# pmvreeswijk/BlackBOX

Hardware: AMD Instinct MI355X
Metric: 10560x10560 fp32 frames/sec end-to-end reduce+ZOGY; % HBM roofline (higher is better)
Workload: dtype f32

## Files before the change

### blackbox_amd/csrc/bbx_canny.hip

```cpp
#include "bbx_common.h"

#define CANNY_MAXR 32

struct canny_par {
    unsigned prefix[4];
    unsigned long long rank[4];
    double p1, p2, low, high;
    float p1f, p2f, den;
    int degenerate;
    double w[CANNY_MAXR + 1];
    int radius;
};

__global__ void k_canny_init(canny_par* p, size_t n, double q1, double q2, const double* __restrict__ w, int radius, unsigned* hist) {
    const int t = threadIdx.x;
    for (int i = t; i < 4 * 4096; i += blockDim.x) hist[i] = 0;
    if (t <= radius) p->w[t] = w[t];
    if (t == 0) {
        const double v1 = (double)(n - 1) * q1, v2 = (double)(n - 1) * q2;
        const unsigned long long l1 = (unsigned long long)floor(v1), l2 = (unsigned long long)floor(v2);
        p->rank[0] = l1; p->rank[1] = l1 + 1 < n ? l1 + 1 : n - 1;
        p->rank[2] = l2; p->rank[3] = l2 + 1 < n ? l2 + 1 : n - 1;
        for (int q = 0; q < 4; q++) p->prefix[q] = 0;
        p->radius = radius; p->degenerate = 0;
    }
}

template <int PASS>
__global__ __launch_bounds__(256) void k_canny_hist(const float* __restrict__ b, size_t n, const canny_par* __restrict__ p,
                                                    unsigned* __restrict__ hist) {
    __shared__ unsigned h[4096];
    for (int i = threadIdx.x; i < 4096; i += blockDim.x) h[i] = 0;
    __syncthreads();
    unsigned pre[4];
#pragma unroll
    for (int q = 0; q < 4; q++) pre[q] = p->prefix[q];
    const size_t n4 = n >> 2, stride = (size_t)gridDim.x * blockDim.x;
    const float4* b4 = (const float4*)b;
    auto count = [&](float f) {
        const unsigned k = f2key(f);
        if (PASS == 0) {
            const unsigned bin = k >> 20;
            bool pending = true;
#pragma unroll
            for (int r = 0; r < 2; r++) {
                const unsigned long long act = __builtin_amdgcn_ballot_w64(pending);
                if (!act) break;
                const int leader = (int)__builtin_ctzll(act);
                const unsigned b0 = (unsigned)__builtin_amdgcn_readlane((int)bin, leader);
                const bool same = pending && bin == b0;
                const unsigned long long m = __builtin_amdgcn_ballot_w64(same);
                if ((int)(threadIdx.x & 63) == leader) atomicAdd(&h[b0], (unsigned)__popcll(m));
                pending = pending && !same;
            }
            if (pending) atomicAdd(&h[bin], 1u);
        } else {
#pragma unroll
            for (int q = 0; q < 4; q++) {
                if (q > 0 && pre[q] == pre[q - 1]) continue;
                if (PASS == 1 && (k >> 20) == pre[q]) atomicAdd(&h[q * 1024 + ((k >> 10) & 1023u)], 1u);
                if (PASS == 2 && (k >> 10) == pre[q]) atomicAdd(&h[q * 1024 + (k & 1023u)], 1u);
            }
        }
    };
    for (size_t i = (size_t)blockIdx.x * blockDim.x + threadIdx.x; i < n4; i += stride) {
        const float4 f = b4[i];
        count(f.x); count(f.y); count(f.z); count(f.w);
    }
    if (blockIdx.x == 0 && threadIdx.x < (n & 3)) count(b[n4 * 4 + threadIdx.x]);
    __syncthreads();
    for (int i = threadIdx.x; i < 4096; i += blockDim.x) if (h[i]) atomicAdd(&hist[i], h[i]);
}

template <int PASS>
__global__ __launch_bounds__(256) void k_canny_scan(canny_par* p, unsigned* hist) {
    __shared__ unsigned sh[4096];
    for (int i = threadIdx.x; i < 4096; i += blockDim.x) sh[i] = hist[i];
    __syncthreads();
    const int q = threadIdx.x >> 6, lane = threadIdx.x & 63;
    int qh = q;
    if (PASS != 0) { while (qh > 0 && p->prefix[qh] == p->prefix[qh - 1]) qh--; }
    __syncthreads();
    const unsigned* h = PASS == 0 ? sh : sh + qh * 1024;
    constexpr int NB = PASS == 0 ? 4096 : 1024, CH = NB / 64;
    unsigned long long mine = 0;
    for (int i = 0; i < CH; i++) mine += h[lane * CH + i];
    unsigned long long incl = mine;
#pragma unroll
// ... 164 lines not shown
        }
        __syncthreads();
        const unsigned nc = ncand;
        for (unsigned t = tid; t < nc; t += 256) {
            const int i = s_cand[t];
            const int ty = i / CT_X, tx = i - ty * CT_X, y = y0 + ty, x = x0 + tx;
            const int r = ty + 1, c = tx + 1;
            double is, js;
            grad(r, c, is, js);
            const double m = sqrt(is * is + js * js);
            if (!(m > 0.0 && m >= low)) continue;
            const double ai = fabs(is), aj = fabs(js);
            const bool same = (is >= 0 && js >= 0) || (is <= 0 && js <= 0), opp = (is <= 0 && js >= 0) || (is >= 0 && js <= 0);
            int sec = 0;
            if (same && ai >= aj) sec = 1;
            if (same && ai <= aj) sec = 2;
            if (opp && ai <= aj) sec = 3;
            if (opp && ai >= aj) sec = 4;
            if (!sec) continue;
            const int dr2 = sec <= 2 ? 1 : -1, dr1 = (sec == 1) ? 1 : (sec == 4 ? -1 : 0), dc1 = (sec == 2 || sec == 3) ? 1 : 0;
            const double w = (sec == 1 || sec == 4) ? aj / ai : ai / aj;
            const bool loc = (mag(r + dr2, c + 1) * w + mag(r + dr1, c + dc1) * (1 - w) <= m) &&
                             (mag(r - dr2, c - 1) * w + mag(r - dr1, c - dc1) * (1 - w) <= m);
            if (loc) { const unsigned k = atomicAdd(&qn, 1u); q[k] = (uint32_t)((size_t)y * nx + x) | (m >= high ? 0x80000000u : 0u); }
        }
        __syncthreads();
        if (tid == 0) ncand = 0;
    }
}

int bbx_cc_filter_list(bbx_ctx* ctx, const uint32_t* d_list, const int32_t* d_cnt, size_t cap, int ny, int nx, const uint8_t* d_flag,
                       int min_size, uint32_t* d_out, int32_t* d_out_cnt, uint32_t out_cap, hipStream_t s);

int bbx_canny_edges(bbx_ctx* ctx, const float* d_bin, int ny, int nx, const double* h_gauss, int radius, double low_frac, double high_frac,
                    int min_size, uint32_t* d_out, int32_t* d_out_cnt, uint32_t out_cap, hipStream_t s) {
    if (radius < 1 || radius > CANNY_MAXR || ny < 3 || nx < 3) return BBX_ERR_ARG;
    const size_t n = (size_t)ny * nx;
    int rc;
    const size_t cap = n / 8 + 4096;
    const size_t o_par = 0, o_hist = 4096, o_w = o_hist + 4 * 4096 * 4, o_tmp = o_w + 1024;
    const size_t o_sm = o_tmp + ((n * 4 + 255) & ~(size_t)255);
    const size_t o_list = o_sm + ((n * 8 + 255) & ~(size_t)255), o_flag = o_list + ((cap * 4 + 255) & ~(size_t)255);
    const size_t total = o_flag + cap + 256;
    char* ws = (char*)bbx_ws(ctx, WS_CANNY, total, &rc); if (rc) return rc;
    canny_par* par = (canny_par*)(ws + o_par); unsigned* hist = (unsigned*)(ws + o_hist); double* d_w = (double*)(ws + o_w);
    float* tmp = (float*)(ws + o_tmp); double* sm = (double*)(ws + o_sm);
    uint32_t* list = (uint32_t*)(ws + o_list); uint8_t* hflag = (uint8_t*)(ws + o_flag);
    int32_t* cnt = &ctx->d_counters[CNT_TMP];
    const double q1 = 4.5 / 100.0, q2 = 93.0 / 100.0;
    BBX_HIP(hipMemcpyAsync(d_w, h_gauss, (size_t)(radius + 1) * 8, hipMemcpyHostToDevice, s));
    BBX_HIP(hipMemsetAsync(cnt, 0, sizeof(int32_t), s));
#ifdef SATV
    const int satv = getenv("BBX_DBG_SAT") ? atoi(getenv("BBX_DBG_SAT")) : 0;
    if (satv >= 5) return BBX_OK;
#endif
    hipLaunchKernelGGL(k_canny_init, dim3(1), dim3(256), 0, s, par, n, q1, q2, d_w, radius, hist);
    hipLaunchKernelGGL(k_canny_hist<0>, dim3(1024), dim3(256), 0, s, d_bin, n, par, hist);
    hipLaunchKernelGGL(k_canny_scan<0>, dim3(1), dim3(256), 0, s, par, hist);
    hipLaunchKernelGGL(k_canny_hist<1>, dim3(1024), dim3(256), 0, s, d_bin, n, par, hist);
    hipLaunchKernelGGL(k_canny_scan<1>, dim3(1), dim3(256), 0, s, par, hist);
    hipLaunchKernelGGL(k_canny_hist<2>, dim3(1024), dim3(256), 0, s, d_bin, n, par, hist);
    hipLaunchKernelGGL(k_canny_scan<2>, dim3(1), dim3(256), 0, s, par, hist);
    hipLaunchKernelGGL(k_canny_params, dim3(1), dim3(64), 0, s, par, n, q1, q2, low_frac, high_frac);
    const dim3 gx((nx + 255) / 256, (ny + GH_ROWS - 1) / GH_ROWS), gv((nx + 255) / 256, (ny + GV_RY - 1) / GV_RY);
#ifdef SATV
    if (satv >= 4) return BBX_OK;
#endif
    if (radius == 12) {
        hipLaunchKernelGGL(k_canny_gauss_v<12>, gv, dim3(256), 0, s, d_bin, ny, nx, par, tmp);
        hipLaunchKernelGGL(k_canny_gauss_h<12>, gx, dim3(256), 0, s, tmp, ny, nx, par, sm);
    } else {
        return BBX_ERR_ARG;
    }
#ifdef SATV
    if (satv >= 3) return BBX_OK;
#endif
    hipLaunchKernelGGL(k_canny_tile, dim3((nx + CT_X - 1) / CT_X, (ny + CT_Y * CT_NT - 1) / (CT_Y * CT_NT)), dim3(256), 0, s, sm, ny, nx, par, list, hflag, cnt,
                       (uint32_t)cap, ctx->d_err);
    BBX_LAUNCH_CHECK();
#ifdef SATV
    if (satv >= 2) return BBX_OK;
#endif
    return bbx_cc_filter_list(ctx, list, cnt, cap, ny, nx, hflag, min_size, d_out, d_out_cnt, out_cap, s);
}

__global__ __launch_bounds__(256) void k_canny_scatter(const uint32_t* __restrict__ list, const int32_t* __restrict__ cnt, uint32_t cap,
                                                       uint8_t* __restrict__ map) {
    const uint32_t n = min((uint32_t)*cnt, cap);
    for (uint32_t e = blockIdx.x * blockDim.x + threadIdx.x; e < n; e += gridDim.x * blockDim.x) map[list[e]] = 1;
}

extern "C" int bbx_canny_edge_map(bbx_ctx* ctx, int ny, int nx, const float* d_img, const double* h_gauss, int gauss_radius,
                                  double low_frac, double high_frac, int min_size, uint8_t* d_map, int32_t* d_count, void* stream) {
    if (!ctx || !d_img || !h_gauss || !d_map || !d_count || ((uintptr_t)d_img) % 16) return BBX_ERR_ARG;
    hipStream_t s = (hipStream_t)stream;
    int rc;
    const size_t n = (size_t)ny * nx, cap = n / 8 + 4096;
    uint32_t* out = (uint32_t*)bbx_ws(ctx, WS_CRLIST, cap * sizeof(uint32_t), &rc); if (rc) return rc;
    BBX_HIP(hipMemsetAsync(d_map, 0, n, s));
    rc = bbx_canny_edges(ctx, d_img, ny, nx, h_gauss, gauss_radius, low_frac, high_frac, min_size, out, d_count, (uint32_t)cap, s);
    if (rc) return rc;
    hipLaunchKernelGGL(k_canny_scatter, dim3(256), dim3(256), 0, s, out, d_count, (uint32_t)cap, d_map);
    BBX_LAUNCH_CHECK();
    return BBX_OK;
}

int bbx_build_flags_canny(void) {
#ifdef SATV
    return 8;
#else
    return 0;
#endif
}
```

### blackbox_amd/csrc/bbx_common.h

```cpp
#pragma once
#include <hip/hip_runtime.h>
#include <hip/hip_ext.h>
#include <stdint.h>
#include <stdio.h>
#include <string.h>
#include "../../include/bbx.h"

#define BBX_WAVE 64

struct bbx_dims {
    int ny_raw, nx_raw, ysz, xsz;
    int dy, dx;
    int os_y, os_x;
    int vos_x0, vos_w;
    int hos_rows;
    int ny, nx;
};

static inline int bbx_make_dims(const bbx_geom* g, bbx_dims* d) {
    if (!g || g->ny_raw <= 0 || g->nx_raw <= 0 || g->ysize_chan <= 0 || g->xsize_chan <= 0)
        return BBX_ERR_ARG;
    d->ny_raw = g->ny_raw; d->nx_raw = g->nx_raw;
    d->ysz = g->ysize_chan; d->xsz = g->xsize_chan;
    if (d->ny_raw % 2 || d->nx_raw % 8) return BBX_ERR_ARG;
    d->dy = d->ny_raw / 2; d->dx = d->nx_raw / 8;
    d->os_y = (d->ny_raw - 2 * d->ysz) / 2;
    d->os_x = (d->nx_raw - 8 * d->xsz) / 8;
    if (d->os_y != d->dy - d->ysz || d->os_x != d->dx - d->xsz) return BBX_ERR_ARG;
    d->hos_rows = d->os_y - 10;
    d->vos_x0 = d->xsz + 5;
    d->vos_w = d->dx - 1 - d->vos_x0;
    if (d->hos_rows <= 0 || d->vos_w <= 0) return BBX_ERR_ARG;
    d->ny = 2 * d->ysz; d->nx = 8 * d->xsz;
    return BBX_OK;
}

#define BBX_DERR_LIST_OVERFLOW 1
#define BBX_DERR_NOTCONV       2
#define BBX_DERR_PSF_WINDOW    4

struct bbx_zprep { const float2* buf; const void* id[2]; int S; int geom[4]; };

struct bbx_ctx {
    int device;
    char hip_err[256];
    int32_t* d_err;
    uint32_t* d_satlist;  int64_t cap_satlist;
    void*     flags_clean_ptr;
    size_t    flags_clean_bytes;
    void*     d_nonlin;
    int       nonlin_on;
    void*     hash_clean_ptr;
    size_t    hash_clean_n;
    int32_t*  d_counters;
    void*  d_ws[24];
    size_t ws_bytes[24];
    int    lac_feed;
    int    debug_listcap;
    void*  zogy_state;
    void*  zogy_frame_state;
    int    zogy_kwin_off;
    int    zogy_ksmall_off;
    int    sat_attr_set;
    int    mini_attr_set;
    float  zcand_thr;
    const float* zcand_img;
    float  zcand_thr_used; size_t zcand_npix;
    bbx_zprep zrows;
    bbx_zprep zpsf;
    const float* bcand_med;
    double bcand_nsig;
    const float* bcand_img;
    const float* bcand_img_med; double bcand_img_nsig; size_t bcand_npix;
    int    wait_sleep_us;
    int    cc_roots;
    int    box_pp;
    int    bkg_full_sort;
    int    fpack_hist_only;
    struct { void* stream; void* ptr; size_t bytes; } fphint[16];
    int    fpack_one_wg;
    int    spf_attr_bytes;
    int    zogy3_attr_L;
    int    num_cus;
    int prof_on, prof_n;
    volatile int prof_gen;
    int prof_open, prof_open_gen, prof_open_idx;
    hipEvent_t* prof_ev;
    int* prof_slot;
};
#define BBX_PROF_MAX 8192
void bbx_prof_start(bbx_ctx* ctx, int slot, hipStream_t s);
void bbx_prof_stop(bbx_ctx* ctx, hipStream_t s);
void bbx_prof_events(bbx_ctx* ctx, int slot, hipEvent_t* e0, hipEvent_t* e1);
#define BBX_LAUNCH_TIMED(ctx, slot, kern, grid, blk, lds, s, ...)                                   \
    do {                                                                                              \
        hipEvent_t e0_ = nullptr, e1_ = nullptr;                                                      \
        bbx_prof_events(ctx, slot, &e0_, &e1_);                                                       \
        hipExtLaunchKernelGGL(kern, grid, blk, lds, s, e0_, e1_, 0, __VA_ARGS__);                     \
    } while (0)

enum {
    CNT_SAT = 0,
    CNT_CAND = 16,
    CNT_STAGE2 = 32,
    CNT_CRLIST = 48,
    CNT_NEWCR = 64,
    CNT_CC_N = 80,
    CNT_CC_ROOTS = 96,
    CNT_TILES = 112,
    CNT_BGNEED = 128,
    CNT_TMP = 144,
    CNT_CANDOVF = 160,
    CNT_CANDRAW = 176,
    CNT_TICKET = 192,
    CNT_ZCAND = 208,
    CNT_BCAND = 224,
    CNT_BOXFAIL0 = 240,
    CNT_MAX = 256
};

enum {
    WS_HASH = 0, WS_CCLIST, WS_PARENT, WS_BITS_M, WS_BITS_C, WS_BITS_R, WS_TILES,
    WS_CAND, WS_FLAGS, WS_STAGE2, WS_CRLIST, WS_HIST, WS_SEL, WS_MISC, WS_STRIP, WS_HVALS, WS_CRORIG, WS_CANNY, WS_ZCAND, WS_BCAND, WS_FPHINT, WS_BOXFAIL, WS_ZSPL,
    WS_TRANSFIT,
    WS_MAX
};

int bbx_hip_fail(bbx_ctx* ctx, hipError_t e, const char* what, int line);
static inline size_t bbx_cand_cap(size_t npix) {
    const size_t c = npix / 16 + 1024, f = npix < 65536 ? npix : 65536;
    return c > f ? c : f;
}
void bbx_zogy_frame_release(bbx_ctx* ctx);
void bbx_fpack_release(bbx_ctx* ctx);
int bbx_build_flags_fpack(void); int bbx_build_flags_zogy(void); int bbx_build_flags_bkg(void); int bbx_build_flags_sat(void); int bbx_build_flags_canny(void);
void bbx_zogy_release(bbx_ctx* ctx);
void* bbx_ws(bbx_ctx* ctx, int slot, size_t bytes, int* rc);

struct f32x16 { float v[16]; };
struct f64x256 { double v[256]; };

#define BBX_HIP(call)                                                         \
    do {                                                                      \
        hipError_t _e = (call);                                               \
        if (_e != hipSuccess) return bbx_hip_fail(ctx, _e, #call, __LINE__);  \
    } while (0)

#define BBX_LAUNCH_CHECK()                                                    \
    do {                                                                      \
        hipError_t _e = hipGetLastError();                                    \
        if (_e != hipSuccess) return bbx_hip_fail(ctx, _e, "kernel launch", __LINE__); \
    } while (0)

template <int CTRL> __device__ __forceinline__ int dpp_mov_i32(int v) {
    return __builtin_amdgcn_update_dpp(0, v, CTRL, 0xf, 0xf, false);
}
template <int CTRL> __device__ __forceinline__ float dpp_mov_f32(float v) {
    return __int_as_float(dpp_mov_i32<CTRL>(__float_as_int(v)));
}
template <int CTRL> __device__ __forceinline__ double dpp_mov_f64(double v) {
    const int lo = dpp_mov_i32<CTRL>(__double2loint(v)), hi = dpp_mov_i32<CTRL>(__double2hiint(v));
    return __hiloint2double(hi, lo);
}
__device__ __forceinline__ double readlane_f64(double v, int lane) {
    return __hiloint2double(__builtin_amdgcn_readlane(__double2hiint(v), lane), __builtin_amdgcn_readlane(__double2loint(v), lane));
}
__device__ __forceinline__ float readlane_f32(float v, int lane) { return __int_as_float(__builtin_amdgcn_readlane(__float_as_int(v), lane)); }
#define BBX_DPP_ROR(n) (0x120 + (n))
__device__ __forceinline__ double wave_sum_f64(double v) {
    v += dpp_mov_f64<BBX_DPP_ROR(1)>(v);
// ... 31 lines not shown
        if (lane == leader) atomicAdd(&size[r0], (unsigned)__popcll(same));
        on = on && root != r0;
        m &= ~same;
    }
}

__device__ __forceinline__ bool finite_f32(float v) { return (__float_as_uint(v) & 0x7f800000u) != 0x7f800000u; }

__device__ __forceinline__ unsigned atomic_or_u8(uint8_t* base, size_t idx, unsigned bits) {
    size_t a = (size_t)(base + idx);
    unsigned* w = (unsigned*)(a & ~(size_t)3);
    unsigned sh = (unsigned)(a & 3) * 8;
    unsigned old = atomicOr(w, bits << sh);
    return (old >> sh) & 0xffu;
}
__device__ __forceinline__ void atomic_clear_u8(uint8_t* base, size_t idx, unsigned bits) {
    size_t a = (size_t)(base + idx);
    atomicAnd((unsigned*)(a & ~(size_t)3), ~(bits << ((unsigned)(a & 3) * 8)));
}

template <int RAW_T>
__device__ __forceinline__ float raw_load(const void* raw, size_t i) {
    if (RAW_T == BBX_RAW_U16) return (float)((const uint16_t*)raw)[i];
    return ((const float*)raw)[i];
}

__device__ __forceinline__ uint32_t f2key(float f) {
    uint32_t u = __float_as_uint(f);
    return (u & 0x80000000u) ? ~u : (u | 0x80000000u);
}
__device__ __forceinline__ float key2f(uint32_t k) {
    uint32_t u = (k & 0x80000000u) ? (k & 0x7fffffffu) : ~k;
    return __uint_as_float(u);
}

__device__ __forceinline__ uint32_t umed3(uint32_t a, uint32_t b, uint32_t c) {
    uint32_t o;
    asm("v_med3_u32 %0, %1, %2, %3" : "=v"(o) : "v"(a), "v"(b), "v"(c));
    return o;
}
template <int NR, int K, int J> __device__ __forceinline__ void wave_sort_static(uint32_t (&k)[NR]) {
#pragma unroll
    for (int r = 0; r < NR; r++) {
        const int q = r ^ J;
        if (q > r) {
            const uint32_t a = k[r], b = k[q];
            const uint32_t lo = min(a, b), hi = max(a, b);
            if ((r & K) == 0) { k[r] = lo; k[q] = hi; } else { k[r] = hi; k[q] = lo; }
        }
    }
}
template <int NR, int J> __device__ __forceinline__ void wave_sort_lane(uint32_t (&k)[NR], uint32_t clo) {
    const uint32_t chi = ~clo;
#pragma unroll
    for (int r = 0; r < NR; r++) {
        const int q = r ^ J;
        if (q > r) {
            const uint32_t a = k[r], b = k[q];
            k[r] = umed3(a, b, clo); k[q] = umed3(a, b, chi);
        }
    }
}
template <int NR> __device__ __forceinline__ void wave_sort_cross(uint32_t (&k)[NR], int lane, int m, bool asc) {
    const uint32_t c = (((lane & m) == 0) == asc) ? 0u : 0xffffffffu;
#pragma unroll
    for (int r = 0; r < NR; r++) k[r] = umed3(k[r], (uint32_t)__shfl_xor((int)k[r], m), c);
// ... 102 lines not shown
```

### blackbox_amd/csrc/bbx_ctx.hip

```cpp
#include "bbx_common.h"
#include <stdlib.h>
#include <time.h>

int bbx_hip_fail(bbx_ctx* ctx, hipError_t e, const char* what, int line) {
    if (ctx)
        snprintf(ctx->hip_err, sizeof(ctx->hip_err), "%s: %s (line %d)", what,
                 hipGetErrorString(e), line);
    (void)hipGetLastError();
    return BBX_ERR_HIP;
}

void* bbx_ws(bbx_ctx* ctx, int slot, size_t bytes, int* rc) {
    *rc = BBX_OK;
    if (slot < 0 || slot >= WS_MAX) { *rc = BBX_ERR_ARG; return nullptr; }
    if (ctx->ws_bytes[slot] >= bytes && ctx->d_ws[slot]) return ctx->d_ws[slot];
    if (ctx->d_ws[slot]) {
        (void)hipDeviceSynchronize();
        (void)hipFree(ctx->d_ws[slot]);
        ctx->d_ws[slot] = nullptr; ctx->ws_bytes[slot] = 0;
    }
    size_t want = bytes + bytes / 8 + 256;
    hipError_t e = hipMalloc(&ctx->d_ws[slot], want);
    if (e != hipSuccess) { *rc = bbx_hip_fail(ctx, e, "hipMalloc(workspace)", __LINE__); return nullptr; }
    ctx->ws_bytes[slot] = want;
    return ctx->d_ws[slot];
}

void bbx_prof_start(bbx_ctx* ctx, int slot, hipStream_t s) {
    ctx->prof_open = 0;
    if (!ctx->prof_on || ctx->prof_n >= BBX_PROF_MAX) return;
    const int n = ctx->prof_n;
    ctx->prof_open_gen = ctx->prof_gen;
    ctx->prof_slot[n] = slot;
    (void)hipEventRecord(ctx->prof_ev[2 * n], s);
    ctx->prof_open = 1; ctx->prof_open_idx = n;
}
void bbx_prof_events(bbx_ctx* ctx, int slot, hipEvent_t* e0, hipEvent_t* e1) {
    *e0 = *e1 = nullptr;
    ctx->prof_open = 0;
    if (!ctx->prof_on || ctx->prof_n >= BBX_PROF_MAX) return;
    const int n = ctx->prof_n;
    ctx->prof_slot[n] = slot;
    *e0 = ctx->prof_ev[2 * n]; *e1 = ctx->prof_ev[2 * n + 1];
    ctx->prof_n = n + 1;
}
void bbx_prof_stop(bbx_ctx* ctx, hipStream_t s) {
    if (!ctx->prof_open) return;
    ctx->prof_open = 0;
    if (!ctx->prof_on || ctx->prof_open_gen != ctx->prof_gen || ctx->prof_open_idx != ctx->prof_n) return;
    (void)hipEventRecord(ctx->prof_ev[2 * ctx->prof_n + 1], s);
    ctx->prof_n++;
}

#define BBX_HIP0(call) do { if ((call) != hipSuccess) return BBX_ERR_HIP; } while (0)

extern "C" {

int bbx_version(void) { return 100; }
// ... 47 lines not shown

int bbx_ctx_create(int device, bbx_ctx** out) {
    if (!out) return BBX_ERR_ARG;
    *out = nullptr;
    bbx_ctx* ctx = (bbx_ctx*)calloc(1, sizeof(bbx_ctx));
    if (!ctx) return BBX_ERR_NOMEM;
    ctx->device = device;
    hipError_t e = hipSetDevice(device);
    if (e == hipSuccess) e = hipMalloc((void**)&ctx->d_err, 4 * sizeof(int32_t));
    if (e == hipSuccess) e = hipMemset(ctx->d_err, 0, 4 * sizeof(int32_t));
    if (e == hipSuccess) e = hipMalloc((void**)&ctx->d_counters, CNT_MAX * sizeof(int32_t));
    if (e == hipSuccess) e = hipMemset(ctx->d_counters, 0, CNT_MAX * sizeof(int32_t));
    ctx->num_cus = 0;
    if (e == hipSuccess) e = hipDeviceGetAttribute(&ctx->num_cus, hipDeviceAttributeMultiprocessorCount, device);
    if (e != hipSuccess) {
        fprintf(stderr, "bbx_ctx_create: %s\n", hipGetErrorString(e));
        free(ctx);
        return BBX_ERR_HIP;
    }
    *out = ctx;
    return BBX_OK;
}

void bbx_ctx_destroy(bbx_ctx* ctx) {
    if (!ctx) return;
    (void)hipSetDevice(ctx->device);
    (void)hipDeviceSynchronize();
    bbx_zogy_release(ctx);
    bbx_zogy_frame_release(ctx);
    bbx_fpack_release(ctx);
    for (int i = 0; i < WS_MAX; i++) if (ctx->d_ws[i]) (void)hipFree(ctx->d_ws[i]);
    if (ctx->d_satlist) (void)hipFree(ctx->d_satlist);
    if (ctx->d_nonlin) (void)hipFree(ctx->d_nonlin);
    if (ctx->d_err) (void)hipFree(ctx->d_err);
    if (ctx->d_counters) (void)hipFree(ctx->d_counters);
    if (ctx->prof_ev) { for (int i = 0; i < 2 * BBX_PROF_MAX; i++) (void)hipEventDestroy(ctx->prof_ev[i]); free(ctx->prof_ev); free(ctx->prof_slot); }
    free(ctx);
}

__global__ __launch_bounds__(256) void k_copy_bytes(const uint8_t* __restrict__ src, uint8_t* __restrict__ dst, size_t n, int words) {
    const size_t i0 = (size_t)blockIdx.x * blockDim.x + threadIdx.x, step = (size_t)gridDim.x * blockDim.x;
    if (words) {
        const size_t nw = n >> 2;
        for (size_t i = i0; i < nw; i += step) reinterpret_cast<uint32_t*>(dst)[i] = reinterpret_cast<const uint32_t*>(src)[i];
        for (size_t i = (nw << 2) + i0; i < n; i += step) dst[i] = src[i];
    } else {
        for (size_t i = i0; i < n; i += step) dst[i] = src[i];
    }
}

int bbx_copy_kernel(void* dst, const void* src, size_t nbytes, void* stream) {
    if (!dst || !src) return BBX_ERR_ARG;
    if (nbytes == 0) return BBX_OK;
    const int words = (((uintptr_t)dst | (uintptr_t)src) & 3) == 0;
    const size_t items = words ? (nbytes >> 2) + 3 : nbytes;
    const int blocks = (int)((items + 255) / 256 < 1024 ? (items + 255) / 256 : 1024);
    hipLaunchKernelGGL(k_copy_bytes, dim3(blocks), dim3(256), 0, (hipStream_t)stream, (const uint8_t*)src, (uint8_t*)dst, nbytes, words);
    if (hipGetLastError() != hipSuccess) return BBX_ERR_HIP;
    return BBX_OK;
}

static int bbx_poll_event(hipEvent_t ev, int sleep_us) {
    struct timespec ts; ts.tv_sec = 0; ts.tv_nsec = (long)sleep_us * 1000L;
    for (;;) {
        const hipError_t e = hipEventQuery(ev);
        if (e == hipSuccess) return BBX_OK;
// ... 29 lines not shown
    int32_t* err = g_wait.h_err;
    err[0] = 0;
    BBX_HIP(hipMemcpyAsync(err, ctx->d_err, 4 * sizeof(int32_t), hipMemcpyDeviceToHost, (hipStream_t)stream));
    { const int rc = bbx_wait(ctx, stream); if (rc) return rc; }
    if (err[0]) {
        BBX_HIP(hipMemsetAsync(ctx->d_err, 0, 4 * sizeof(int32_t), (hipStream_t)stream));
        if (err[0] & BBX_DERR_PSF_WINDOW) return BBX_ERR_PSFWIN;
        if (err[0] & BBX_DERR_LIST_OVERFLOW) return BBX_ERR_OVERFLOW;
        if (err[0] & BBX_DERR_NOTCONV) return BBX_ERR_NOTCONV;
    }
    return BBX_OK;
}

__global__ void k_step_mark(int32_t* err, int32_t* slot) { *slot = err[0]; err[0] = 0; }

int bbx_step_mark(bbx_ctx* ctx, int32_t* d_slot, void* stream) {
    if (!ctx || !d_slot) return BBX_ERR_ARG;
    hipLaunchKernelGGL(k_step_mark, dim3(1), dim3(1), 0, (hipStream_t)stream, ctx->d_err, d_slot);
    BBX_LAUNCH_CHECK();
    return BBX_OK;
}

int bbx_set_option(bbx_ctx* ctx, int option, int value) {
    if (!ctx) return BBX_ERR_ARG;
    if (option == BBX_OPT_LAC_LEVEL_FEED) { ctx->lac_feed = value ? 1 : 0; return BBX_OK; }
    if (option == BBX_OPT_ZOGY_CORE) return BBX_OK;
    if (option == BBX_OPT_DEBUG_LISTCAP) { ctx->debug_listcap = value > 0 ? value : 0; return BBX_OK; }
    if (option == BBX_OPT_ZOGY_KWIN_OFF) { ctx->zogy_kwin_off = value ? 1 : 0; return BBX_OK; }
    if (option == BBX_OPT_ZOGY_KSMALL_OFF) { ctx->zogy_ksmall_off = value ? 1 : 0; return BBX_OK; }
    if (option == BBX_OPT_FPACK_ONE_WG) { ctx->fpack_one_wg = value ? 1 : 0; return BBX_OK; }
    if (option == BBX_OPT_FPACK_HIST_ONLY) { ctx->fpack_hist_only = value ? 1 : 0; return BBX_OK; }
    if (option == BBX_OPT_BKG_FULL_SORT) { ctx->bkg_full_sort = value ? 1 : 0; return BBX_OK; }
    if (option == BBX_OPT_WAIT_SLEEP_US) { ctx->wait_sleep_us = value > 0 ? value : 0; return BBX_OK; }
    return BBX_ERR_ARG;
}


int bbx_event_create(void** out_event) {
    if (!out_event) return BBX_ERR_ARG;
    hipEvent_t ev;
    BBX_HIP0(hipEventCreateWithFlags(&ev, hipEventDisableTiming));
    *out_event = (void*)ev;
    return BBX_OK;
}

void bbx_event_destroy(void* event) {
    if (event) (void)hipEventDestroy((hipEvent_t)event);
}

int bbx_event_record(void* event, void* stream) {
    if (!event) return BBX_ERR_ARG;
    BBX_HIP0(hipEventRecord((hipEvent_t)event, (hipStream_t)stream));
    return BBX_OK;
}

int bbx_event_query(void* event) {
    if (!event) return BBX_ERR_ARG;
    const hipError_t e = hipEventQuery((hipEvent_t)event);
    if (e == hipSuccess) return 1;
    if (e == hipErrorNotReady) { (void)hipGetLastError(); return 0; }
    return BBX_ERR_HIP;
}

int bbx_stream_wait_event(void* stream, void* event) {
    if (!event) return BBX_ERR_ARG;
    BBX_HIP0(hipStreamWaitEvent((hipStream_t)stream, (hipEvent_t)event, 0));
// ... 13 lines not shown
```

### blackbox_amd/csrc/bbx_sat.hip

```cpp
#include "bbx_common.h"

#define SAT_BLOCKS 1024

struct sat_state {
    unsigned long long best;
    int accept, found, k, lo_off, hi_off;
    int votes;
    double rho, c, s, chord;
    unsigned long long tmin, tmax;
    double t0, t1;
    unsigned long long fit_n; long long fit_t, fit_d, fit_tt, fit_td;
    double icpt, slope;
    unsigned int bmax_key, bmin_key;
    int seg[4], seg_ok;
    double m[6], m2[6];
    int rot_rows, rot_cols, back_rows, back_cols, crop_y, crop_x;
    double sx, sy;
    double top, clip_lo, clip_hi;
    int band_r0, band_rows;
    int nwin, row_min, row_max;
};
#define SAT_BANDH 96
#define SAT_MAXWIN 1200
#define SAT_SEG_CAP 8192
#define SAT_SUBLEN 5
#define SAT_SUBW 200
struct sat_rect { int r0, r1, c0, c1; };


__global__ __launch_bounds__(256) void k_bin2(const float* __restrict__ d, int nyb, int nxb, float* __restrict__ b) {
    const int X = blockIdx.x * blockDim.x + threadIdx.x, Y = blockIdx.y;
    if (X >= nxb) return;
    const size_t nx = (size_t)nxb * 2;
    const float2 r0 = *(const float2*)(d + (size_t)(2 * Y) * nx + 2 * X);
    const float2 r1 = *(const float2*)(d + (size_t)(2 * Y + 1) * nx + 2 * X);
    b[(size_t)Y * nxb + X] = (r0.x + r0.y) + (r1.x + r1.y);
}

__global__ __launch_bounds__(256) void k_bin_minmax(const float* __restrict__ b, size_t n, sat_state* st) {
    unsigned hi = 0u, lo = ~0u;
    const size_t n4 = n >> 2, stride = (size_t)gridDim.x * blockDim.x;
    const float4* b4 = (const float4*)b;
    for (size_t i = (size_t)blockIdx.x * blockDim.x + threadIdx.x; i < n4; i += stride) {
        const float4 q = b4[i];
        const float f[4] = {q.x, q.y, q.z, q.w};
#pragma unroll
        for (int u = 0; u < 4; u++) if (isfinite(f[u])) { const unsigned k = f2key(f[u]); hi = k > hi ? k : hi; lo = k < lo ? k : lo; }
    }
    if (blockIdx.x == 0 && threadIdx.x < (n & 3)) { const float f = b[(n4 << 2) + threadIdx.x]; if (isfinite(f)) { const unsigned k = f2key(f); hi = k > hi ? k : hi; lo = k < lo ? k : lo; } }
    for (int o = 32; o > 0; o >>= 1) { const unsigned a = __shfl_xor(hi, o, 64), c = __shfl_xor(lo, o, 64); hi = a > hi ? a : hi; lo = c < lo ? c : lo; }
    __shared__ unsigned shi[4], slo[4];
    if ((threadIdx.x & 63) == 0) { shi[threadIdx.x >> 6] = hi; slo[threadIdx.x >> 6] = lo; }
    __syncthreads();
    if (threadIdx.x == 0) {
        for (int w = 1; w < 4; w++) { hi = shi[w] > hi ? shi[w] : hi; lo = slo[w] < lo ? slo[w] : lo; }
        if (hi) { atomicMax(&st->bmax_key, hi); atomicMin(&st->bmin_key, lo); }
    }
}

__global__ void k_sat_init(sat_state* st) {
    if (threadIdx.x == 0) {
        st->best = 0;
        st->accept = 0; st->found = 0; st->k = 0; st->lo_off = 0; st->hi_off = 0; st->votes = 0;
        st->rho = 0; st->c = 0; st->s = 0; st->chord = 0; st->tmin = ~0ull; st->tmax = 0ull; st->t0 = 0; st->t1 = 0;
        st->fit_n = 0; st->fit_t = st->fit_d = st->fit_tt = st->fit_td = 0; st->icpt = 0; st->slope = 0;
        st->bmax_key = 0u; st->bmin_key = ~0u; st->seg_ok = 0; st->nwin = 0; st->row_min = 0x7fffffff; st->row_max = -1;
        st->band_r0 = 0; st->band_rows = 0; st->rot_rows = st->rot_cols = 0;
    }
}

__global__ __launch_bounds__(1024) void k_hough_lds(const uint32_t* __restrict__ list, const int32_t* __restrict__ cnt, uint32_t cap,
                                                    int nxb, const double* __restrict__ cs, int nrho, sat_state* st) {
    extern __shared__ unsigned hist[];
    const int k = blockIdx.x;
    const uint32_t n = min((uint32_t)*cnt, cap);
    for (int i = threadIdx.x; i < nrho; i += blockDim.x) hist[i] = 0;
    __syncthreads();
    const double c = cs[2 * k], s = cs[2 * k + 1];
    const int off = nrho / 2;
    for (uint32_t e = threadIdx.x; e < n; e += blockDim.x) {
        const uint32_t p = list[e];
        const double y = (double)(p / nxb), x = (double)(p % nxb);
        const double r = c * x + s * y;
        atomicAdd(&hist[(int)(r > 0.0 ? r + 0.5 : r - 0.5) + off], 1u);
    }
    __syncthreads();
    unsigned long long best = 0;
    for (int i = threadIdx.x; i < nrho; i += blockDim.x) {
        const unsigned v = hist[i];
        const unsigned long long flat = (unsigned long long)k * nrho + i;
// ... 392 lines not shown
        const double fminr = floor(r), fminc = floor(c);
        const long long minr = (long long)fminr, minc = (long long)fminc, maxr = (long long)ceil(r), maxc = (long long)ceil(c);
        const double dr = r - fminr, dc = c - fminc;
        double p[4];
        const long long rr[4] = {minr, minr, maxr, maxr}, cc[4] = {minc, maxc, minc, maxc};
        for (int q = 0; q < 4; q++) {
            double v = 0.0;
            if (rr[q] >= 0 && rr[q] < rot_rows && cc[q] >= 0 && cc[q] < rot_cols)
                for (int w = 0; w < nwin; w++)
                    if (rr[q] >= R[w].r0 && rr[q] < R[w].r1 && cc[q] >= R[w].c0 && cc[q] < R[w].c1) { v = 1.0; break; }
            p[q] = v;
        }
        const double top = (1 - dc) * p[0] + dc * p[1], bot = (1 - dc) * p[2] + dc * p[3];
        const double out = (1 - dr) * top + dr * bot;
        if (out != 0.0) {
            uint16_t* a = reinterpret_cast<uint16_t*>(mask + (size_t)(2 * Y) * nx + 2 * X);
            uint16_t* bq = reinterpret_cast<uint16_t*>(mask + (size_t)(2 * Y + 1) * nx + 2 * X);
            *a |= (uint16_t)(BBX_MASK_SATELLITE | (BBX_MASK_SATELLITE << 8));
            *bq |= (uint16_t)(BBX_MASK_SATELLITE | (BBX_MASK_SATELLITE << 8));
        }
    }
}

__global__ void k_sat_info(const sat_state* __restrict__ st, float* info) {
    if (threadIdx.x == 0) {
        info[0] = key2f(st->bmax_key); info[1] = key2f(st->bmin_key); info[2] = (float)st->votes; info[3] = (float)st->k;
        info[4] = (float)st->rho; info[5] = (float)st->nwin; info[6] = (float)st->seg_ok; info[7] = (float)st->found;
    }
}

extern "C" int bbx_count_objects(bbx_ctx* ctx, int ny, int nx, const uint8_t* d_mask, int bit, int32_t* d_count, void* stream);

int bbx_canny_edges(bbx_ctx* ctx, const float* d_bin, int ny, int nx, const double* h_gauss, int radius, double low_frac, double high_frac,
                    int min_size, uint32_t* d_out, int32_t* d_out_cnt, uint32_t out_cap, hipStream_t s);

extern "C" int bbx_sat_trails(bbx_ctx* ctx, int ny, int nx, const float* d_data, uint8_t* d_mask, const double* h_cos_sin,
                              int ntheta, const double* h_gauss, int gauss_radius, int32_t* d_nsats, float* d_info, void* stream) {
    if (!ctx || !d_data || !d_mask || !h_cos_sin || !h_gauss || !d_nsats || !d_info || ny < 8 || nx < 8 || (ny & 1) || (nx & 1) ||
        ntheta < 4 || ntheta > 4096 || ((uintptr_t)d_data) % 8)
        return BBX_ERR_ARG;
    hipStream_t s = (hipStream_t)stream;
    const int nyb = ny / 2, nxb = nx / 2;
    const size_t nb = (size_t)nyb * nxb;
    const int nrho = 2 * (int)ceil(sqrt((double)nyb * nyb + (double)nxb * nxb));
    int rc;
    const size_t cap = nb / 8 + 4096;
    const size_t o_bin = 0, o_list = o_bin + ((nb * 4 + 255) & ~(size_t)255);
    const size_t o_cs = o_list + ((cap * 4 + 255) & ~(size_t)255), o_part = o_cs + (((size_t)ntheta * 16 + 255) & ~(size_t)255);
    const size_t o_st = o_part + SAT_BLOCKS * 3 * 8;
    const int band_cols = nrho / 2 + 8;
    const size_t o_rect = (o_st + sizeof(sat_state) + 255) & ~(size_t)255, o_band = (o_rect + SAT_MAXWIN * sizeof(sat_rect) + 255) & ~(size_t)255;
    const size_t total = o_band + (size_t)2 * SAT_BANDH * band_cols * sizeof(double) + 256;
    char* ws = (char*)bbx_ws(ctx, WS_CAND, total, &rc); if (rc) return rc;
    float* bin = (float*)(ws + o_bin); uint32_t* list = (uint32_t*)(ws + o_list);
    double* cs = (double*)(ws + o_cs); sat_state* st = (sat_state*)(ws + o_st);
    sat_rect* rects = (sat_rect*)(ws + o_rect); double* band = (double*)(ws + o_band);
    int32_t* cnt = &ctx->d_counters[CNT_CAND];
    BBX_HIP(hipMemcpyAsync(cs, h_cos_sin, (size_t)ntheta * 16, hipMemcpyHostToDevice, s));
    hipLaunchKernelGGL(k_sat_init, dim3(1), dim3(128), 0, s, st);
    hipLaunchKernelGGL(k_bin2, dim3((nxb + 255) / 256, nyb), dim3(256), 0, s, d_data, nyb, nxb, bin);
    hipLaunchKernelGGL(k_bin_minmax, dim3(1024), dim3(256), 0, s, bin, nb, st);
    rc = bbx_canny_edges(ctx, bin, nyb, nxb, h_gauss, gauss_radius, 0.1, 0.2, 60, list, cnt, (uint32_t)cap, s); if (rc) return rc;
#ifdef SATV
    if (getenv("BBX_DBG_SAT") && atoi(getenv("BBX_DBG_SAT")) >= 1) return BBX_OK;
#endif
    if ((size_t)nrho * 4 <= 150 * 1024) {
        hipLaunchKernelGGL(k_hough_lds, dim3(ntheta), dim3(1024), (size_t)nrho * 4, s, list, cnt, (uint32_t)cap, nxb, cs, nrho, st);
    } else {
        return BBX_ERR_ARG;
    }
    hipLaunchKernelGGL(k_trail_decide, dim3(1), dim3(64), 0, s, st, cs, nrho, nyb, nxb, 210);
    const double refine_tol[4] = {0.0, 3.0, 2.0, 1.5};
    for (int it = 0; it < 4; it++) {
        hipLaunchKernelGGL(k_trail_cone, dim3(256), dim3(256), 0, s, list, cnt, (uint32_t)cap, nxb, st, refine_tol[it]);
        hipLaunchKernelGGL(k_trail_refine, dim3(1), dim3(64), 0, s, st);
    }
    hipLaunchKernelGGL(k_trail_support, dim3(256), dim3(256), 0, s, list, cnt, (uint32_t)cap, nxb, st);
    hipLaunchKernelGGL(k_trail_accept, dim3(1), dim3(64), 0, s, st, 40.0);
    const size_t seg_lds = (size_t)SAT_SEG_CAP * 12;
    if (ctx->sat_attr_set != 1) {
        BBX_HIP(hipFuncSetAttribute((const void*)k_trail_segment, hipFuncAttributeMaxDynamicSharedMemorySize, (int)seg_lds));
        ctx->sat_attr_set = 1;
    }
    hipLaunchKernelGGL(k_trail_segment, dim3(1), dim3(1024), seg_lds, s, list, cnt, (uint32_t)cap, nyb, nxb, nrho, st, ctx->d_err);
    hipLaunchKernelGGL(k_sat_rotband, dim3((band_cols + 255) / 256, 2 * SAT_BANDH), dim3(256), 0, s, bin, nyb, nxb, st, band, band_cols);
    hipLaunchKernelGGL(k_sat_walk, dim3(1), dim3(256), 0, s, band, band_cols, st, rects, ctx->d_err);
    hipLaunchKernelGGL(k_sat_paint, dim3(2048), dim3(256), 0, s, d_mask, nyb, nxb, st, rects);
    hipLaunchKernelGGL(k_sat_info, dim3(1), dim3(64), 0, s, st, d_info);
    BBX_LAUNCH_CHECK();
    return bbx_count_objects(ctx, ny, nx, d_mask, BBX_MASK_SATELLITE, d_nsats, stream);
}

int bbx_build_flags_sat(void) {
#ifdef SATV
    return 8;
// ... 5 lines not shown
```

### include/bbx.h

```cpp
#ifndef BBX_H
#define BBX_H

#include <stddef.h>
#include <stdint.h>

#ifdef __cplusplus
extern "C" {
#endif

#define BBX_OK            0
#define BBX_ERR_ARG      -1
#define BBX_ERR_HIP      -2
#define BBX_ERR_NOMEM    -3
#define BBX_ERR_OVERFLOW -4
#define BBX_ERR_NOTCONV  -5
#define BBX_ERR_PSFWIN   -6

#define BBX_NCHAN 16

#define BBX_MASK_BAD        1
#define BBX_MASK_COSMIC     2
#define BBX_MASK_SAT        4
#define BBX_MASK_SATCON     8
#define BBX_MASK_SATELLITE 16
#define BBX_MASK_EDGE      32
#define BBX_MASK_XTALK     64

#define BBX_RAW_U16 0
#define BBX_RAW_F32 1

typedef struct bbx_ctx bbx_ctx;

typedef struct {
    int32_t ny_raw, nx_raw;
    int32_t ysize_chan, xsize_chan;
} bbx_geom;

int  bbx_ctx_create(int device, bbx_ctx **out);
void bbx_ctx_destroy(bbx_ctx *ctx);
const char *bbx_strerror(int code);
const char *bbx_last_hip_error(const bbx_ctx *ctx);
int  bbx_version(void);
int  bbx_build_flags(void);
int  bbx_sync(bbx_ctx *ctx, void *stream);

#define BBX_OPT_LAC_LEVEL_FEED 1
#define BBX_OPT_DEBUG_LISTCAP 2
#define BBX_OPT_ZOGY_CORE 3
#define BBX_OPT_ZOGY_KWIN_OFF 4
#define BBX_OPT_FPACK_ONE_WG 5
#define BBX_OPT_FPACK_HIST_ONLY 6
#define BBX_OPT_WAIT_SLEEP_US 7
#define BBX_OPT_BKG_FULL_SORT 8
#define BBX_OPT_ZOGY_KSMALL_OFF 9
int  bbx_set_option(bbx_ctx *ctx, int option, int value);
int  bbx_wait(bbx_ctx *ctx, void *stream);
int  bbx_copy_kernel(void *dst, const void *src, size_t nbytes, void *stream);
int  bbx_event_wait(void *event, int sleep_us);

int  bbx_step_mark(bbx_ctx *ctx, int32_t *d_slot, void *stream);

int  bbx_event_create(void **out_event);
void bbx_event_destroy(void *event);
int  bbx_event_record(void *event, void *stream);
int  bbx_event_query(void *event);
int  bbx_stream_wait_event(void *stream, void *event);
int  bbx_copy_async(void *dst, const void *src, size_t nbytes, int kind, void *stream);

#define BBX_PROF_CALIBRATE 0
#define BBX_PROF_LAC_DENSE 1
#define BBX_PROF_LAC_SPARSE 2
#define BBX_PROF_XTALK 3
#define BBX_PROF_VOS_STD 4
#define BBX_PROF_MASK_FINISH 5
#define BBX_PROF_ZOGY 6
#define BBX_PROF_ZOGY_FINAL 7
#define BBX_PROF_Z_PSF_COLS 8
#define BBX_PROF_Z_PSF_ROWS 9
#define BBX_PROF_Z_IMG_ROWS 10
#define BBX_PROF_Z_IMG_COLS 11
#define BBX_PROF_Z_VAR_COLS 12
#define BBX_PROF_Z_PSF_DFT 13
#define BBX_PROF_NSLOTS 14
int  bbx_profile_enable(bbx_ctx *ctx, int on);
int  bbx_profile_read(bbx_ctx *ctx, double *ms_total, int32_t *calls, int nslots);

int bbx_overscan_stats(bbx_ctx *ctx, const bbx_geom *g, const void *d_raw,
// ... 261 lines not shown
```

Baseline: 144.8.

## Fuse 2x2 binning, min/max and canny pass-0 histogram; cache constant tables

```diff
diff --git a/blackbox_amd/csrc/bbx_canny.hip b/blackbox_amd/csrc/bbx_canny.hip
--- a/blackbox_amd/csrc/bbx_canny.hip
+++ b/blackbox_amd/csrc/bbx_canny.hip
@@ -40,20 +40,7 @@
     auto count = [&](float f) {
         const unsigned k = f2key(f);
         if (PASS == 0) {
-            const unsigned bin = k >> 20;
-            bool pending = true;
-#pragma unroll
-            for (int r = 0; r < 2; r++) {
-                const unsigned long long act = __builtin_amdgcn_ballot_w64(pending);
-                if (!act) break;
-                const int leader = (int)__builtin_ctzll(act);
-                const unsigned b0 = (unsigned)__builtin_amdgcn_readlane((int)bin, leader);
-                const bool same = pending && bin == b0;
-                const unsigned long long m = __builtin_amdgcn_ballot_w64(same);
-                if ((int)(threadIdx.x & 63) == leader) atomicAdd(&h[b0], (unsigned)__popcll(m));
-                pending = pending && !same;
-            }
-            if (pending) atomicAdd(&h[bin], 1u);
+            lds_hist_add_wave(h, k >> 20);
         } else {
 #pragma unroll
             for (int q = 0; q < 4; q++) {
@@ -284,30 +271,52 @@
 int bbx_cc_filter_list(bbx_ctx* ctx, const uint32_t* d_list, const int32_t* d_cnt, size_t cap, int ny, int nx, const uint8_t* d_flag,
                        int min_size, uint32_t* d_out, int32_t* d_out_cnt, uint32_t out_cap, hipStream_t s);
 
-int bbx_canny_edges(bbx_ctx* ctx, const float* d_bin, int ny, int nx, const double* h_gauss, int radius, double low_frac, double high_frac,
-                    int min_size, uint32_t* d_out, int32_t* d_out_cnt, uint32_t out_cap, hipStream_t s) {
-    if (radius < 1 || radius > CANNY_MAXR || ny < 3 || nx < 3) return BBX_ERR_ARG;
+struct canny_ws { canny_par* par; unsigned* hist; float* tmp; double* sm; uint32_t* list; uint8_t* hflag; size_t cap; };
+static int canny_workspace(bbx_ctx* ctx, int ny, int nx, canny_ws* o) {
     const size_t n = (size_t)ny * nx;
     int rc;
     const size_t cap = n / 8 + 4096;
-    const size_t o_par = 0, o_hist = 4096, o_w = o_hist + 4 * 4096 * 4, o_tmp = o_w + 1024;
+    const size_t o_par = 0, o_hist = 4096, o_tmp = o_hist + 4 * 4096 * 4 + 1024;
     const size_t o_sm = o_tmp + ((n * 4 + 255) & ~(size_t)255);
     const size_t o_list = o_sm + ((n * 8 + 255) & ~(size_t)255), o_flag = o_list + ((cap * 4 + 255) & ~(size_t)255);
     const size_t total = o_flag + cap + 256;
     char* ws = (char*)bbx_ws(ctx, WS_CANNY, total, &rc); if (rc) return rc;
-    canny_par* par = (canny_par*)(ws + o_par); unsigned* hist = (unsigned*)(ws + o_hist); double* d_w = (double*)(ws + o_w);
-    float* tmp = (float*)(ws + o_tmp); double* sm = (double*)(ws + o_sm);
-    uint32_t* list = (uint32_t*)(ws + o_list); uint8_t* hflag = (uint8_t*)(ws + o_flag);
+    o->par = (canny_par*)(ws + o_par); o->hist = (unsigned*)(ws + o_hist);
+    o->tmp = (float*)(ws + o_tmp); o->sm = (double*)(ws + o_sm);
+    o->list = (uint32_t*)(ws + o_list); o->hflag = (uint8_t*)(ws + o_flag); o->cap = cap;
+    return BBX_OK;
+}
+static const double CANNY_Q1 = 4.5 / 100.0, CANNY_Q2 = 93.0 / 100.0;
+
+int bbx_canny_begin(bbx_ctx* ctx, int ny, int nx, const double* h_gauss, int radius, hipStream_t s, unsigned** hist) {
+    if (radius < 1 || radius > CANNY_MAXR || ny < 3 || nx < 3) return BBX_ERR_ARG;
+    canny_ws w;
+    int rc = canny_workspace(ctx, ny, nx, &w); if (rc) return rc;
+    const double* d_w = (const double*)bbx_const_table(ctx, CTAB_CANNY_GAUSS, h_gauss, (size_t)(radius + 1) * 8, s, &rc); if (rc) return rc;
+    hipLaunchKernelGGL(k_canny_init, dim3(1), dim3(256), 0, s, w.par, (size_t)ny * nx, CANNY_Q1, CANNY_Q2, d_w, radius, w.hist);
+    BBX_LAUNCH_CHECK();
+    if (hist) *hist = w.hist;
+    return BBX_OK;
+}
+
+int bbx_canny_edges(bbx_ctx* ctx, const float* d_bin, int ny, int nx, const double* h_gauss, int radius, double low_frac, double high_frac,
+                    int min_size, uint32_t* d_out, int32_t* d_out_cnt, uint32_t out_cap, hipStream_t s, int pass0_done) {
+    if (radius < 1 || radius > CANNY_MAXR || ny < 3 || nx < 3) return BBX_ERR_ARG;
+    const size_t n = (size_t)ny * nx;
+    int rc;
+    if (!pass0_done) { rc = bbx_canny_begin(ctx, ny, nx, h_gauss, radius, s, nullptr); if (rc) return rc; }
+    canny_ws w;
+    rc = canny_workspace(ctx, ny, nx, &w); if (rc) return rc;
+    canny_par* par = w.par; unsigned* hist = w.hist; float* tmp = w.tmp; double* sm = w.sm;
+    uint32_t* list = w.list; uint8_t* hflag = w.hflag; const size_t cap = w.cap;
     int32_t* cnt = &ctx->d_counters[CNT_TMP];
-    const double q1 = 4.5 / 100.0, q2 = 93.0 / 100.0;
-    BBX_HIP(hipMemcpyAsync(d_w, h_gauss, (size_t)(radius + 1) * 8, hipMemcpyHostToDevice, s));
+    const double q1 = CANNY_Q1, q2 = CANNY_Q2;
     BBX_HIP(hipMemsetAsync(cnt, 0, sizeof(int32_t), s));
 #ifdef SATV
     const int satv = getenv("BBX_DBG_SAT") ? atoi(getenv("BBX_DBG_SAT")) : 0;
     if (satv >= 5) return BBX_OK;
 #endif
-    hipLaunchKernelGGL(k_canny_init, dim3(1), dim3(256), 0, s, par, n, q1, q2, d_w, radius, hist);
-    hipLaunchKernelGGL(k_canny_hist<0>, dim3(1024), dim3(256), 0, s, d_bin, n, par, hist);
+    if (!pass0_done) hipLaunchKernelGGL(k_canny_hist<0>, dim3(1024), dim3(256), 0, s, d_bin, n, par, hist);
     hipLaunchKernelGGL(k_canny_scan<0>, dim3(1), dim3(256), 0, s, par, hist);
     hipLaunchKernelGGL(k_canny_hist<1>, dim3(1024), dim3(256), 0, s, d_bin, n, par, hist);
     hipLaunchKernelGGL(k_canny_scan<1>, dim3(1), dim3(256), 0, s, par, hist);
@@ -350,7 +359,7 @@
     const size_t n = (size_t)ny * nx, cap = n / 8 + 4096;
     uint32_t* out = (uint32_t*)bbx_ws(ctx, WS_CRLIST, cap * sizeof(uint32_t), &rc); if (rc) return rc;
     BBX_HIP(hipMemsetAsync(d_map, 0, n, s));
-    rc = bbx_canny_edges(ctx, d_img, ny, nx, h_gauss, gauss_radius, low_frac, high_frac, min_size, out, d_count, (uint32_t)cap, s);
+    rc = bbx_canny_edges(ctx, d_img, ny, nx, h_gauss, gauss_radius, low_frac, high_frac, min_size, out, d_count, (uint32_t)cap, s, 0);
     if (rc) return rc;
     hipLaunchKernelGGL(k_canny_scatter, dim3(256), dim3(256), 0, s, out, d_count, (uint32_t)cap, d_map);
     BBX_LAUNCH_CHECK();
diff --git a/blackbox_amd/csrc/bbx_common.h b/blackbox_amd/csrc/bbx_common.h
--- a/blackbox_amd/csrc/bbx_common.h
+++ b/blackbox_amd/csrc/bbx_common.h
@@ -40,6 +40,8 @@
 #define BBX_DERR_PSF_WINDOW    4
 
 struct bbx_zprep { const float2* buf; const void* id[2]; int S; int geom[4]; };
+
+enum { CTAB_SAT_COSSIN = 0, CTAB_CANNY_GAUSS, CTAB_MAX };
 
 struct bbx_ctx {
     int device;
@@ -82,6 +84,8 @@
     int    spf_attr_bytes;
     int    zogy3_attr_L;
     int    num_cus;
+    int    sat_front_split;
+    struct { void* d; void* h; size_t bytes, cap; } ctab[CTAB_MAX];
     int prof_on, prof_n;
     volatile int prof_gen;
     int prof_open, prof_open_gen, prof_open_idx;
@@ -136,6 +140,7 @@
 int bbx_build_flags_fpack(void); int bbx_build_flags_zogy(void); int bbx_build_flags_bkg(void); int bbx_build_flags_sat(void); int bbx_build_flags_canny(void);
 void bbx_zogy_release(bbx_ctx* ctx);
 void* bbx_ws(bbx_ctx* ctx, int slot, size_t bytes, int* rc);
+const void* bbx_const_table(bbx_ctx* ctx, int which, const void* h, size_t bytes, hipStream_t s, int* rc);
 
 struct f32x16 { float v[16]; };
 struct f64x256 { double v[256]; };
@@ -233,6 +238,22 @@
 __device__ __forceinline__ float key2f(uint32_t k) {
     uint32_t u = (k & 0x80000000u) ? (k & 0x7fffffffu) : ~k;
     return __uint_as_float(u);
+}
+
+__device__ __forceinline__ void lds_hist_add_wave(unsigned* h, unsigned bin) {
+    bool pending = true;
+#pragma unroll
+    for (int r = 0; r < 2; r++) {
+        const unsigned long long act = __builtin_amdgcn_ballot_w64(pending);
+        if (!act) break;
+        const int leader = (int)__builtin_ctzll(act);
+        const unsigned b0 = (unsigned)__builtin_amdgcn_readlane((int)bin, leader);
+        const bool same = pending && bin == b0;
+        const unsigned long long m = __builtin_amdgcn_ballot_w64(same);
+        if ((int)(threadIdx.x & 63) == leader) atomicAdd(&h[b0], (unsigned)__popcll(m));
+        pending = pending && !same;
+    }
+    if (pending) atomicAdd(&h[bin], 1u);
 }
 
 __device__ __forceinline__ uint32_t umed3(uint32_t a, uint32_t b, uint32_t c) {
diff --git a/blackbox_amd/csrc/bbx_ctx.hip b/blackbox_amd/csrc/bbx_ctx.hip
--- a/blackbox_amd/csrc/bbx_ctx.hip
+++ b/blackbox_amd/csrc/bbx_ctx.hip
@@ -24,6 +24,29 @@
     if (e != hipSuccess) { *rc = bbx_hip_fail(ctx, e, "hipMalloc(workspace)", __LINE__); return nullptr; }
     ctx->ws_bytes[slot] = want;
     return ctx->d_ws[slot];
+}
+
+const void* bbx_const_table(bbx_ctx* ctx, int which, const void* h, size_t bytes, hipStream_t s, int* rc) {
+    *rc = BBX_OK;
+    if (which < 0 || which >= CTAB_MAX || !h || !bytes) { *rc = BBX_ERR_ARG; return nullptr; }
+    auto& t = ctx->ctab[which];
+    if (t.d && t.bytes == bytes && !memcmp(t.h, h, bytes)) return t.d;
+    if (t.cap < bytes) {
+        if (t.d) { (void)hipDeviceSynchronize(); (void)hipFree(t.d); }
+        free(t.h);
+        t.d = nullptr; t.h = nullptr; t.bytes = t.cap = 0;
+        t.h = malloc(bytes);
+        if (!t.h) { *rc = BBX_ERR_NOMEM; return nullptr; }
+        hipError_t e = hipMalloc(&t.d, bytes);
+        if (e != hipSuccess) { free(t.h); t.h = nullptr; t.d = nullptr; *rc = bbx_hip_fail(ctx, e, "hipMalloc(table)", __LINE__); return nullptr; }
+        t.cap = bytes;
+    }
+    t.bytes = 0;
+    memcpy(t.h, h, bytes);
+    hipError_t e = hipMemcpyAsync(t.d, t.h, bytes, hipMemcpyHostToDevice, s);
+    if (e != hipSuccess) { *rc = bbx_hip_fail(ctx, e, "hipMemcpyAsync(table)", __LINE__); return nullptr; }
+    t.bytes = bytes;
+    return t.d;
 }
 
 void bbx_prof_start(bbx_ctx* ctx, int slot, hipStream_t s) {
@@ -137,6 +160,7 @@
     for (int i = 0; i < WS_MAX; i++) if (ctx->d_ws[i]) (void)hipFree(ctx->d_ws[i]);
     if (ctx->d_satlist) (void)hipFree(ctx->d_satlist);
     if (ctx->d_nonlin) (void)hipFree(ctx->d_nonlin);
+    for (int i = 0; i < CTAB_MAX; i++) { if (ctx->ctab[i].d) (void)hipFree(ctx->ctab[i].d); free(ctx->ctab[i].h); }
     if (ctx->d_err) (void)hipFree(ctx->d_err);
     if (ctx->d_counters) (void)hipFree(ctx->d_counters);
     if (ctx->prof_ev) { for (int i = 0; i < 2 * BBX_PROF_MAX; i++) (void)hipEventDestroy(ctx->prof_ev[i]); free(ctx->prof_ev); free(ctx->prof_slot); }
@@ -232,6 +256,7 @@
     if (option == BBX_OPT_FPACK_HIST_ONLY) { ctx->fpack_hist_only = value ? 1 : 0; return BBX_OK; }
     if (option == BBX_OPT_BKG_FULL_SORT) { ctx->bkg_full_sort = value ? 1 : 0; return BBX_OK; }
     if (option == BBX_OPT_WAIT_SLEEP_US) { ctx->wait_sleep_us = value > 0 ? value : 0; return BBX_OK; }
+    if (option == BBX_OPT_SAT_FRONT_SPLIT) { ctx->sat_front_split = value ? 1 : 0; return BBX_OK; }
     return BBX_ERR_ARG;
 }
 
diff --git a/blackbox_amd/csrc/bbx_sat.hip b/blackbox_amd/csrc/bbx_sat.hip
--- a/blackbox_amd/csrc/bbx_sat.hip
+++ b/blackbox_amd/csrc/bbx_sat.hip
@@ -56,6 +56,41 @@
         for (int w = 1; w < 4; w++) { hi = shi[w] > hi ? shi[w] : hi; lo = slo[w] < lo ? slo[w] : lo; }
         if (hi) { atomicMax(&st->bmax_key, hi); atomicMin(&st->bmin_key, lo); }
     }
+}
+
+#define BS_BLOCKS 2048
+__global__ __launch_bounds__(256) void k_bin2_stats(const float* __restrict__ d, int nyb, int nxb, float* __restrict__ b, sat_state* st,
+                                                    unsigned* __restrict__ hist) {
+    __shared__ unsigned h[4096];
+    __shared__ unsigned shi[4], slo[4];
+    for (int i = threadIdx.x; i < 4096; i += blockDim.x) h[i] = 0;
+    __syncthreads();
+    const unsigned nq = (unsigned)nxb >> 2;
+    const unsigned total = (unsigned)nyb * nq, stride = gridDim.x * blockDim.x;
+    const size_t nx = (size_t)nxb * 2;
+    unsigned hi = 0u, lo = ~0u;
+    for (unsigned g = blockIdx.x * blockDim.x + threadIdx.x; g < total; g += stride) {
+        const unsigned Y = g / nq, X = g - Y * nq;
+        const float4* p0 = (const float4*)(d + (size_t)(2 * Y) * nx + 8 * X);
+        const float4* p1 = (const float4*)(d + (size_t)(2 * Y + 1) * nx + 8 * X);
+        const float4 a0 = p0[0], a1 = p0[1], c0 = p1[0], c1 = p1[1];
+        const float f[4] = {(a0.x + a0.y) + (c0.x + c0.y), (a0.z + a0.w) + (c0.z + c0.w), (a1.x + a1.y) + (c1.x + c1.y), (a1.z + a1.w) + (c1.z + c1.w)};
+        *(float4*)(b + (size_t)Y * nxb + 4 * X) = make_float4(f[0], f[1], f[2], f[3]);
+#pragma unroll
+        for (int u = 0; u < 4; u++) {
+            const unsigned k = f2key(f[u]);
+            if (isfinite(f[u])) { hi = k > hi ? k : hi; lo = k < lo ? k : lo; }
+            lds_hist_add_wave(h, k >> 20);
+        }
+    }
+    for (int o = 32; o > 0; o >>= 1) { const unsigned a = __shfl_xor(hi, o, 64), c = __shfl_xor(lo, o, 64); hi = a > hi ? a : hi; lo = c < lo ? c : lo; }
+    if ((threadIdx.x & 63) == 0) { shi[threadIdx.x >> 6] = hi; slo[threadIdx.x >> 6] = lo; }
+    __syncthreads();
+    if (threadIdx.x == 0) {
+        for (int w = 1; w < 4; w++) { hi = shi[w] > hi ? shi[w] : hi; lo = slo[w] < lo ? slo[w] : lo; }
+        if (hi) { atomicMax(&st->bmax_key, hi); atomicMin(&st->bmin_key, lo); }
+    }
+    for (int i = threadIdx.x; i < 4096; i += blockDim.x) if (h[i]) atomicAdd(&hist[i], h[i]);
 }
 
 __global__ void k_sat_init(sat_state* st) {
@@ -514,7 +549,8 @@
 extern "C" int bbx_count_objects(bbx_ctx* ctx, int ny, int nx, const uint8_t* d_mask, int bit, int32_t* d_count, void* stream);
 
 int bbx_canny_edges(bbx_ctx* ctx, const float* d_bin, int ny, int nx, const double* h_gauss, int radius, double low_frac, double high_frac,
-                    int min_size, uint32_t* d_out, int32_t* d_out_cnt, uint32_t out_cap, hipStream_t s);
+                    int min_size, uint32_t* d_out, int32_t* d_out_cnt, uint32_t out_cap, hipStream_t s, int pass0_done);
+int bbx_canny_begin(bbx_ctx* ctx, int ny, int nx, const double* h_gauss, int radius, hipStream_t s, unsigned** hist);
 
 extern "C" int bbx_sat_trails(bbx_ctx* ctx, int ny, int nx, const float* d_data, uint8_t* d_mask, const double* h_cos_sin,
                               int ntheta, const double* h_gauss, int gauss_radius, int32_t* d_nsats, float* d_info, void* stream) {
@@ -528,21 +564,30 @@
     int rc;
     const size_t cap = nb / 8 + 4096;
     const size_t o_bin = 0, o_list = o_bin + ((nb * 4 + 255) & ~(size_t)255);
-    const size_t o_cs = o_list + ((cap * 4 + 255) & ~(size_t)255), o_part = o_cs + (((size_t)ntheta * 16 + 255) & ~(size_t)255);
+    const size_t o_part = o_list + ((cap * 4 + 255) & ~(size_t)255);
     const size_t o_st = o_part + SAT_BLOCKS * 3 * 8;
     const int band_cols = nrho / 2 + 8;
     const size_t o_rect = (o_st + sizeof(sat_state) + 255) & ~(size_t)255, o_band = (o_rect + SAT_MAXWIN * sizeof(sat_rect) + 255) & ~(size_t)255;
     const size_t total = o_band + (size_t)2 * SAT_BANDH * band_cols * sizeof(double) + 256;
     char* ws = (char*)bbx_ws(ctx, WS_CAND, total, &rc); if (rc) return rc;
     float* bin = (float*)(ws + o_bin); uint32_t* list = (uint32_t*)(ws + o_list);
-    double* cs = (double*)(ws + o_cs); sat_state* st = (sat_state*)(ws + o_st);
+    sat_state* st = (sat_state*)(ws + o_st);
     sat_rect* rects = (sat_rect*)(ws + o_rect); double* band = (double*)(ws + o_band);
     int32_t* cnt = &ctx->d_counters[CNT_CAND];
-    BBX_HIP(hipMemcpyAsync(cs, h_cos_sin, (size_t)ntheta * 16, hipMemcpyHostToDevice, s));
+    const double* cs = (const double*)bbx_const_table(ctx, CTAB_SAT_COSSIN, h_cos_sin, (size_t)ntheta * 16, s, &rc); if (rc) return rc;
+    const bool fused = !ctx->sat_front_split && nx % 8 == 0 && ((uintptr_t)d_data) % 16 == 0 && ((uintptr_t)bin) % 16 == 0;
+    unsigned* hist = nullptr;
+    if (fused) { rc = bbx_canny_begin(ctx, nyb, nxb, h_gauss, gauss_radius, s, &hist); if (rc) return rc; }
     hipLaunchKernelGGL(k_sat_init, dim3(1), dim3(128), 0, s, st);
-    hipLaunchKernelGGL(k_bin2, dim3((nxb + 255) / 256, nyb), dim3(256), 0, s, d_data, nyb, nxb, bin);
-    hipLaunchKernelGGL(k_bin_minmax, dim3(1024), dim3(256), 0, s, bin, nb, st);
-    rc = bbx_canny_edges(ctx, bin, nyb, nxb, h_gauss, gauss_radius, 0.1, 0.2, 60, list, cnt, (uint32_t)cap, s); if (rc) return rc;
+    if (fused) {
+        const size_t groups = nb / 4;
+        hipLaunchKernelGGL(k_bin2_stats, dim3((unsigned)((groups + 255) / 256 < BS_BLOCKS ? (groups + 255) / 256 : BS_BLOCKS)), dim3(256), 0, s, d_data, nyb, nxb,
+                           bin, st, hist);
+    } else {
+        hipLaunchKernelGGL(k_bin2, dim3((nxb + 255) / 256, nyb), dim3(256), 0, s, d_data, nyb, nxb, bin);
+        hipLaunchKernelGGL(k_bin_minmax, dim3(1024), dim3(256), 0, s, bin, nb, st);
+    }
+    rc = bbx_canny_edges(ctx, bin, nyb, nxb, h_gauss, gauss_radius, 0.1, 0.2, 60, list, cnt, (uint32_t)cap, s, fused ? 1 : 0); if (rc) return rc;
 #ifdef SATV
     if (getenv("BBX_DBG_SAT") && atoi(getenv("BBX_DBG_SAT")) >= 1) return BBX_OK;
 #endif
diff --git a/include/bbx.h b/include/bbx.h
--- a/include/bbx.h
+++ b/include/bbx.h
@@ -53,6 +53,7 @@
 #define BBX_OPT_WAIT_SLEEP_US 7
 #define BBX_OPT_BKG_FULL_SORT 8
 #define BBX_OPT_ZOGY_KSMALL_OFF 9
+#define BBX_OPT_SAT_FRONT_SPLIT 10
 int  bbx_set_option(bbx_ctx *ctx, int option, int value);
 int  bbx_wait(bbx_ctx *ctx, void *stream);
 int  bbx_copy_kernel(void *dst, const void *src, size_t nbytes, void *stream);
```

After: 144.8. About the same (-0.0%).
